# iden3/circom

Measured on NVIDIA H100. Metric: witnesses/s, higher is better.
Workload: dtype u256 (8x u32 limbs, Montgomery)

## Files before the change

### circom_b200/csrc/flatten.cpp

```cpp
#include <algorithm>
#include <bitset>
#include <cstdio>
#include <cstdlib>
#include <cstring>
#include <functional>
#include <stdexcept>
#include <unordered_map>

#include "../../include/circom_b200.h"
#include "tape.h"

namespace cw {

uint64_t fnv1a(const char *s, size_t n) {
    uint64_t h = 0xCBF29CE484222325ULL;
    for (size_t i = 0; i < n; ++i) {
        h ^= (uint64_t)(int64_t)(signed char)s[i];
        h *= 0x100000001B3ULL;
    }
    return h;
}

namespace {

enum { K_NONE = 0, K_OWN = 1, K_SUB = 2, K_CONST = 3, K_TMP = 4, K_ONE = 5 };
enum Form { FC = 0, FM = 1, FD = 2 };

struct IrOp {
    uint32_t op;
    uint64_t d, a, b, c;
};
struct Term {
    uint64_t ref;
    uint32_t cid;
};
struct Tmpl {
    std::string name;
    uint32_t n_out, n_in, n_inter, n_tmp, n_own;
    std::vector<uint32_t> subs;
    std::vector<IrOp> ops;
    std::vector<uint32_t> lc_len;
    std::vector<Term> terms;
    std::vector<uint8_t> tmp_zero_only;
    uint64_t total_signals = 0, total_components = 0;
};

inline int rk(uint64_t r) { return (int)(r >> 56); }
inline uint32_t rsub(uint64_t r) { return (uint32_t)((r >> 32) & 0xFFFFFF); }
inline uint32_t ridx(uint64_t r) { return (uint32_t)r; }

struct Reader {
    const uint8_t *p, *end;
    template <class T>
    T get() {
        if (p + sizeof(T) > end) throw std::runtime_error("cb2c: truncated");
        T v;
        memcpy(&v, p, sizeof(T));
        p += sizeof(T);
        return v;
    }
    const uint8_t *bytes(size_t n) {
        if (n > (size_t)(end - p)) throw std::runtime_error("cb2c: truncated");
        const uint8_t *r = p;
        p += n;
        return r;
    }
    size_t left() const { return (size_t)(end - p); }
    void expect(uint64_t count, uint64_t bytes_each) const {
        if (count * bytes_each > left()) throw std::runtime_error("cb2c: truncated (count exceeds the file)");
    }
    std::string str() {
        uint32_t n = get<uint32_t>();
        const uint8_t *b = bytes((size_t)(((uint64_t)n + 3) & ~3ull));
        return std::string((const char *)b, n);
    }
};

struct Val {
    uint32_t slot[3] = {NO_SLOT, NO_SLOT, NO_SLOT};
    int32_t cid = -1;
    uint16_t bits = 256;
    uint8_t org_op = 0;
    int32_t org_a = -1, org_b = -1;
    int32_t fld_src = -1, bf_src = -1;
    uint16_t fld_k = 0, fld_m = 0, bf_lo = 0, bf_len = 0;
};

enum { DOP_BITS = 29, DOP_ASSERT_BOOL = 30, DOP_MULSMALL = 31, DOP_BITSIP = 32, DOP_ASSERT_FITS = 33 };
enum { DOP_ADDI = 48, DOP_SHRK = 49, DOP_SHLK = 50, DOP_ADDI_H = 52, DOP_MULI_Q = 53, DOP_MULI_H = 54, DOP_SHRK_H = 55,
       DOP_SHLK_H = 56 };
inline bool c_is_immediate(uint32_t opcode) {
    return opcode == CW_OP_ASSERT || opcode == CW_OP_ASSERT_EQ || opcode == DOP_BITS || opcode == DOP_ASSERT_BOOL ||
           opcode == DOP_BITSIP || opcode == DOP_ASSERT_FITS;
}
inline bool is_assert_op(uint32_t opcode) {
    return opcode == CW_OP_ASSERT || opcode == CW_OP_ASSERT_EQ || opcode == DOP_ASSERT_BOOL || opcode == DOP_ASSERT_FITS;
}

inline size_t n_live_ops(const std::vector<uint8_t> &live, uint32_t n_pre, size_t n_prov) {
    size_t n = 0;
    for (size_t i = 0; i < n_prov; ++i) n += live[n_pre + i];
    return n;
}
inline int subtree_need(uint32_t i, const std::vector<uint32_t> &kid_a, const std::vector<uint32_t> &kid_b) {
    const uint32_t a = kid_a[i], b = kid_b[i];
    if (a == NO_SLOT && b == NO_SLOT) return 1;
    if (a == NO_SLOT) return subtree_need(b, kid_a, kid_b);
    if (b == NO_SLOT) return subtree_need(a, kid_a, kid_b);
    const int na = subtree_need(a, kid_a, kid_b), nb = subtree_need(b, kid_a, kid_b);
    return std::max(std::max(na, nb), std::min(na, nb) + 1);
}

static uint32_t coalesce_function_copies(uint32_t *code, uint32_t n_instr, uint32_t n_regs, const std::vector<uint32_t> &fn_params) {
    constexpr uint32_t MAXR = 192;
    if (n_regs > MAXR || n_instr < 2) return n_instr;
    using Set = std::bitset<MAXR>;
    enum { JMP = 40, JZ = 41, RET = 42, LOADX = 43, STOREX = 44, CALLF = 45, COPY = 24 };
    auto is_reg = [&](uint32_t o) { return !(o & 0xC0000000u) && o < n_regs; };
    Set pinned;
    std::vector<uint8_t> target(n_instr + 1, 0);
    for (uint32_t i = 0; i < n_instr; ++i) {
        const uint32_t *w = &code[5 * (size_t)i];
        uint32_t lo = 0, hi = 0;
        if (w[0] == LOADX) { lo = w[2] & 0x3FFFFFFFu; hi = w[4] & 0x3FFFFFFFu; }
        else if (w[0] == STOREX) { lo = w[2] & 0x3FFFFFFFu; hi = w[1] & 0x3FFFFFFFu; }
        else if (w[0] == RET && (w[3] & 0x3FFFFFFFu) > 1) { lo = w[2]; hi = lo + (w[3] & 0x3FFFFFFFu); }
        else if (w[0] == CALLF) {
            for (uint32_t r = w[3]; r < w[3] + fn_params[w[2] & 0x3FFFFFFFu] && r < n_regs; ++r) pinned.set(r);
            if ((w[4] & 0x3FFFFFFFu) > 1) { lo = w[1]; hi = lo + (w[4] & 0x3FFFFFFFu); }
        }
        for (uint32_t r = lo; r < hi && r < n_regs; ++r) pinned.set(r);
        if (w[0] == JMP) target[std::min(w[2] & 0x3FFFFFFFu, n_instr)] = 1;
        if (w[0] == JZ) target[std::min(w[3] & 0x3FFFFFFFu, n_instr)] = 1;
    }
    std::vector<Set> use(n_instr), live_in(n_instr), live_out(n_instr);
    std::vector<int> def(n_instr, -1);
    auto add_use = [&](uint32_t i, uint32_t o) { if (is_reg(o) && !pinned.test(o)) use[i].set(o); };
    for (uint32_t i = 0; i < n_instr; ++i) {
        const uint32_t *w = &code[5 * (size_t)i];
        switch (w[0]) {
            case JMP: break;
            case JZ: add_use(i, w[2]); break;
            case RET: if ((w[3] & 0x3FFFFFFFu) <= 1) add_use(i, w[2]); break;
            case LOADX: add_use(i, w[3]); if (!pinned.test(w[1])) def[i] = (int)w[1]; break;
            case STOREX: add_use(i, w[3]); add_use(i, w[4]); break;
            case CALLF: if (!pinned.test(w[1])) def[i] = (int)w[1]; break;
            default: add_use(i, w[2]); add_use(i, w[3]); add_use(i, w[4]); if (!pinned.test(w[1])) def[i] = (int)w[1];
        }
    }
    for (bool changed = true; changed;) {
        changed = false;
        for (uint32_t i = n_instr; i-- > 0;) {
            const uint32_t *w = &code[5 * (size_t)i];
            Set out;
            if (w[0] == JMP) out = live_in[w[2] & 0x3FFFFFFFu];
            else if (w[0] != RET) {
                if (i + 1 < n_instr) out = live_in[i + 1];
                if (w[0] == JZ) out |= live_in[w[3] & 0x3FFFFFFFu];
            }
            Set in = out;
            if (def[i] >= 0) in.reset((size_t)def[i]);
            in |= use[i];
            if (in != live_in[i] || out != live_out[i]) { live_in[i] = in; live_out[i] = out; changed = true; }
        }
    }
    std::vector<uint8_t> dead(n_instr, 0);
    for (uint32_t i = 1; i < n_instr; ++i) {
        uint32_t *c = &code[5 * (size_t)i], *p = &code[5 * (size_t)(i - 1)];
        if (c[0] != COPY || target[i] || dead[i - 1]) continue;
        const uint32_t t = c[2], d = c[1];
        if (!is_reg(t) || pinned.test(t) || t == d || def[i - 1] != (int)t || live_out[i].test(t)) continue;
        if (p[0] == JMP || p[0] == JZ || p[0] == RET || p[0] == STOREX) continue;
// ... 1349 lines not shown
                }
                ext[i] = e;
                gsig[i] = sg * 1099511628211ull;
                if (!fusedf[i]) {
                    glevel[n_pre + i] = e + 1;
                    max_level = std::max(max_level, e + 1);
                    ++n_roots;
                }
            }
        }
        std::vector<uint32_t> order;
        order.reserve(n_roots);
        for (size_t i = 0; i < n_prov; ++i)
            if (live[n_pre + i] && !fusedf[i] && pops[i * 4] != 47) order.push_back((uint32_t)i);
        std::stable_sort(order.begin(), order.end(), [&](uint32_t x, uint32_t y) {
            uint32_t lx = glevel[n_pre + x], ly = glevel[n_pre + y];
            if (lx != ly) return lx < ly;
            if (pops[x * 4] != pops[y * 4]) return pops[x * 4] < pops[y * 4];
            return gsig[x] < gsig[y];
        });
        std::vector<uint32_t> remap(n_pre + n_prov, NO_SLOT);
        uint32_t next_tmp = (uint32_t)W;
        for (uint32_t i = 0; i < n_pre; ++i) {
            if (claimed[i] < 0) throw std::runtime_error("lowering: main input outside the witness");
            remap[i] = (uint32_t)claimed[i];
        }
        for (size_t r = 0; r < order.size(); ++r) {
            uint32_t p = n_pre + order[r];
            if (claimed[p] >= 0) remap[p] = (uint32_t)claimed[p];
            else if (!is_assert_op(pops[(size_t)order[r] * 4])) remap[p] = next_tmp++;
            if (pops[(size_t)order[r] * 4] == 45) {
                const uint32_t *ct = &pcalls[pops[(size_t)order[r] * 4 + 1]];
                const uint32_t *ex = ct + 2 + ct[1];
                for (uint32_t k = 0; k < ex[0]; ++k) {
                    const uint32_t s = ex[1 + k];
                    if (!live[s]) continue;
                    remap[s] = claimed[s] >= 0 ? (uint32_t)claimed[s] : next_tmp++;
                }
            }
        }
        if (next_tmp >= DST_ACC) throw std::runtime_error("circuit too large for the packed tape word (2^24 slots)");
        T.ops.clear();
        T.ops.reserve(n_live_ops(live, n_pre, n_prov) * 4);
        T.items.clear();
        T.items.reserve(n_roots + 1);
        T.level_start.assign(max_level + 1, 0);
        T.n_mul_ops = 0;
        uint32_t prev_level = 0;
        const bool narrow_on = !(flags & (CW_FLAG_NO_NARROW | CW_FLAG_NO_PEEPHOLE));
        auto opd_bits = [&](uint32_t o) -> uint32_t {
            if (o == NO_SLOT) return 0;
            if (o & OPERAND_CONST) return (uint32_t)u256_bitlen(consts[o & 0x7FFFFFFFu]);
            return o < slot_bits.size() ? slot_bits[o] : 256u;
        };
        auto const_amount = [&](uint32_t o, uint32_t &k) {
            if (o == NO_SLOT || !(o & OPERAND_CONST)) return false;
            const U256 &c = consts[o & 0x7FFFFFFFu];
            if (c.v[1] | c.v[2] | c.v[3] || c.v[0] >= qb()) return false;
            k = (uint32_t)c.v[0];
            return true;
        };
        auto narrow_opcode = [&](uint32_t i) -> uint32_t {
            const uint32_t *o = &pops[(size_t)i * 4];
            if (!narrow_on) return o[0];
            const uint32_t rb = slot_bits[n_pre + i], ba = opd_bits(o[1]), bb = opd_bits(o[2]), lim = qb() - 1;
            uint32_t k;
            switch (o[0]) {
                case CW_OP_ADD:
                    if (rb >= 256 || std::max(ba, bb) + 1 > lim) return o[0];
                    return std::max(ba, bb) + 1 <= 128 ? DOP_ADDI_H : DOP_ADDI;
                case DOP_MULSMALL:
                    if (ba <= 64 && bb <= 64) return DOP_MULI_Q;
                    if (ba <= 128 && bb <= 128) return DOP_MULI_H;
                    return o[0];
                case CW_OP_SHR:
                    if (!const_amount(o[2], k)) return o[0];
                    return ba <= 128 ? DOP_SHRK_H : DOP_SHRK;
                case CW_OP_SHL:
                    if (!const_amount(o[2], k) || ba + k > lim) return o[0];
                    return ba <= 128 ? DOP_SHLK_H : DOP_SHLK;
                default: return o[0];
            }
        };
        for (uint64_t &x : T.width_census) x = 0;
        auto census = [&](uint32_t i, uint32_t opcode) {
            const uint32_t *o = &pops[(size_t)i * 4];
            uint32_t w = is_assert_op(o[0]) ? 0u : slot_bits[n_pre + i];
            for (int k = 1; k <= 3; ++k) {
                if (k == 3 && c_is_immediate(o[0])) break;
                if (o[k] != NO_SLOT && !(o[k] & OPERAND_CONST)) w = std::max(w, opd_bits(o[k]));
            }
            T.width_census[4 * (opcode & 63u) + (w <= 64 ? 0 : w <= 128 ? 1 : w <= 192 ? 2 : 3)]++;
        };
        auto word = [&](uint32_t i, uint32_t dstfield, int acc_a, int acc_b, uint32_t d[4]) {
            const uint32_t *o = &pops[(size_t)i * 4];
            const uint32_t opcode = o[0] == 45 ? o[0] : narrow_opcode(i);
            d[0] = opcode | (dstfield << 8);
            if (o[0] == 45) {
                uint32_t n = pcalls[o[1] + 1];
                d[1] = (uint32_t)T.call_tab.size();
                d[2] = d[3] = OPERAND_CONST;
                T.call_tab.push_back(pcalls[o[1]]);
                T.call_tab.push_back(n);
                for (uint32_t k = 0; k < n; ++k) {
                    uint32_t a = pcalls[o[1] + 2 + k];
                    T.call_tab.push_back((a & OPERAND_CONST) ? a : remap[a]);
                }
                const uint32_t *ex = &pcalls[o[1] + 2 + n];
                T.call_tab.push_back(ex[0]);
                for (uint32_t k = 0; k < ex[0]; ++k) T.call_tab.push_back(live[ex[1 + k]] ? remap[ex[1 + k]] : NO_SLOT);
                return;
            }
            for (int k = 1; k <= 3; ++k) {
                if (k == 3 && c_is_immediate(o[0])) d[k] = o[k];
                else if (o[k] == NO_SLOT) d[k] = OPERAND_CONST;
                else if (o[k] & OPERAND_CONST) d[k] = o[k];
                else if (k == 1 && acc_a >= 0) d[k] = OPERAND_ACC | (uint32_t)acc_a;
                else if (k == 2 && acc_b >= 0) d[k] = OPERAND_ACC | (uint32_t)acc_b;
                else d[k] = remap[o[k]];
            }
        };
        std::function<void(uint32_t, int)> emit_sub = [&](uint32_t i, int target) {
            const uint32_t ka = kid_a[i], kb = kid_b[i];
            int acc_a = -1, acc_b = -1;
            if (ka != NO_SLOT && kb != NO_SLOT) {
                const bool a_first = subtree_need(ka, kid_a, kid_b) >= subtree_need(kb, kid_a, kid_b);
                if (a_first) { emit_sub(ka, target); emit_sub(kb, target ^ 1); }
                else { emit_sub(kb, target); emit_sub(ka, target ^ 1); }
                acc_a = a_first ? target : (target ^ 1);
                acc_b = a_first ? (target ^ 1) : target;
            } else if (ka != NO_SLOT) { emit_sub(ka, target); acc_a = target; }
            else if (kb != NO_SLOT) { emit_sub(kb, target); acc_b = target; }
            uint32_t d[4];
            word(i, DST_ACC + (uint32_t)target, acc_a, acc_b, d);
            census(i, d[0] & 0xFFu);
            T.ops.insert(T.ops.end(), d, d + 4);
            if (pops[(size_t)i * 4] == CW_OP_MUL) ++T.n_mul_ops;
        };
        for (size_t r = 0; r < order.size(); ++r) {
            const uint32_t i = order[r];
            const uint32_t *o = &pops[(size_t)i * 4];
            const uint32_t lvl = glevel[n_pre + i];
            const uint32_t dst = is_assert_op(o[0]) ? 0u : remap[n_pre + i];
            const uint32_t ka = kid_a[i], kb = kid_b[i];
            const bool single = ka == NO_SLOT && kb == NO_SLOT;
            uint32_t d[4];
            if (single) {
                word(i, dst, -1, -1, d);
                if (o[0] == DOP_BITS && !(flags & CW_FLAG_NO_PEEPHOLE) && lvl == prev_level && !T.ops.empty() &&
                    T.items.back() == T.ops.size() / 4 - 1) {
                    uint32_t *p = &T.ops[T.ops.size() - 4];
                    if ((p[0] & 0xFFu) == DOP_BITS && p[1] == d[1] && ((p[3] >> 16) & 0xFFu) == 1u && ((d[3] >> 16) & 0xFFu) == 1u) {
                        uint32_t cnt = (p[3] >> 24) + 1u, pk = p[3] & 0xFFFFu, pdst = p[0] >> 8;
                        if (cnt < 32u && (d[3] & 0xFFFFu) == pk + cnt && dst == pdst + cnt) {
                            p[3] += 1u << 24;
                            continue;
                        }
                    }
                }
                if (o[0] != 45) census(i, d[0] & 0xFFu);
                T.items.push_back((uint32_t)(T.ops.size() / 4));
                T.ops.insert(T.ops.end(), d, d + 4);
            } else {
                T.items.push_back((uint32_t)(T.ops.size() / 4));
                int acc_a = -1, acc_b = -1;
                if (ka != NO_SLOT && kb != NO_SLOT) {
                    const bool a_first = subtree_need(ka, kid_a, kid_b) >= subtree_need(kb, kid_a, kid_b);
                    if (a_first) { emit_sub(ka, 0); emit_sub(kb, 1); }
                    else { emit_sub(kb, 0); emit_sub(ka, 1); }
                    acc_a = a_first ? 0 : 1;
                    acc_b = a_first ? 1 : 0;
                } else if (ka != NO_SLOT) { emit_sub(ka, 0); acc_a = 0; }
                else { emit_sub(kb, 0); acc_b = 0; }
                word(i, dst, acc_a, acc_b, d);
                census(i, d[0] & 0xFFu);
                T.ops.insert(T.ops.end(), d, d + 4);
            }
            prev_level = lvl;
            if (o[0] == CW_OP_MUL) ++T.n_mul_ops;
            T.level_start[lvl]++;
        }
        T.items.push_back((uint32_t)(T.ops.size() / 4));
        {
            std::vector<uint32_t> ls(max_level + 1, 0);
            uint32_t acc = 0;
            uint64_t widest = 0;
            for (uint32_t l = 1; l <= max_level; ++l) {
                ls[l - 1] = acc;
                widest = std::max<uint64_t>(widest, T.level_start[l]);
                acc += T.level_start[l];
            }
            ls[max_level] = acc;
            T.level_start.swap(ls);
            T.max_level_width = widest;
        }
        std::vector<uint32_t> newid;
        T.n_bitwords = 0;
        if (flags & CW_FLAG_BITPLANE) {
            std::vector<uint32_t> code(next_tmp, NO_SLOT);
            uint32_t n_words = 0;
            const size_t n_ops = T.ops.size() / 4;
            for (size_t i = 0; i < n_ops; ++i) {
                const uint32_t *o = &T.ops[i * 4];
                if ((o[0] & 0xFFu) != DOP_BITS || !(o[3] >> 24)) continue;
                const uint32_t run = (o[3] >> 24) + 1u, d0 = o[0] >> 8;
                for (uint32_t j = 0; j < run; ++j) code[d0 + j] = OPERAND_BIT | (n_words * 32u + j);
                ++n_words;
            }
            bool ok = n_words > 0 && n_words < (1u << 24);
            for (size_t i = 0; ok && i < n_ops; ++i) {
                const uint32_t *o = &T.ops[i * 4];
                if ((o[0] & 0xFFu) == DOP_BITS && (o[3] >> 24) && !(o[1] & OPERAND_CONST) && code[o[1]] != NO_SLOT) ok = false;
            }
            for (uint32_t i = 0; ok && i < M.n_in + 1; ++i)
                if (code[remap[i]] != NO_SLOT) ok = false;
            if (next_tmp >= OPERAND_BIT) ok = false;
            if (ok) {
                newid.resize(next_tmp);
                uint32_t nw = 0;
                for (uint32_t s = 0; s < next_tmp; ++s) newid[s] = code[s] == NO_SLOT ? nw++ : code[s];
                uint32_t word = 0;
                for (size_t i = 0; i < n_ops; ++i) {
                    uint32_t *o = &T.ops[i * 4];
                    const uint32_t opc = o[0] & 0xFFu;
                    if (opc == DOP_BITS && (o[3] >> 24)) o[0] = opc | (word++ << 8);
                    else if (!is_assert_op(opc) && (o[0] >> 8) < DST_ACC) o[0] = opc | (newid[o[0] >> 8] << 8);
                    if (opc == 45) continue;
                    for (int k = 1; k <= 3; ++k) {
                        if (k == 3 && c_is_immediate(opc)) break;
                        if (!(o[k] & (OPERAND_CONST | OPERAND_ACC))) o[k] = newid[o[k]];
                    }
                }
                for (size_t i = 0; i < T.call_tab.size();) {
                    const uint32_t n = T.call_tab[i + 1], nx = T.call_tab[i + 2 + n];
                    for (uint32_t k = 0; k < n + 1 + nx; ++k) {
                        if (k == n) continue;
                        uint32_t &e = T.call_tab[i + 2 + k];
                        if (!(e & OPERAND_CONST)) e = newid[e];
                    }
                    i += 3 + n + nx;
                }
                T.n_bitwords = n_words;
                next_tmp = nw;
            }
        }
        const uint32_t n_resident = newid.empty() ? (uint32_t)W : [&]() {
            uint32_t n = 0;
            for (uint64_t i = 0; i < W; ++i) n += !(newid[i] & OPERAND_BIT);
            return n;
        }();
        if (flags & CW_FLAG_REUSE) {
            const size_t n_ops = T.ops.size() / 4;
            const size_t n_lv = T.level_start.size() - 1;
            std::vector<uint32_t> last(next_tmp, 0), phys(next_tmp, NO_SLOT);
            auto is_tmp = [&](uint32_t o) { return !(o & (OPERAND_CONST | OPERAND_BIT | OPERAND_ACC)) && o >= n_resident; };
            for (size_t l = 0; l < n_lv; ++l)
                for (uint32_t i = T.items[T.level_start[l]]; i < T.items[T.level_start[l + 1]]; ++i) {
                    const uint32_t *o = &T.ops[(size_t)i * 4];
                    const uint32_t opc = o[0] & 0xFFu;
                    if (opc == 45) {
                        const uint32_t n = T.call_tab[o[1] + 1];
                        for (uint32_t k = 0; k < n; ++k)
                            if (is_tmp(T.call_tab[o[1] + 2 + k])) last[T.call_tab[o[1] + 2 + k]] = (uint32_t)l;
                        continue;
                    }
// ... 79 lines not shown
        }
        T.witness_slot.resize(W);
        for (uint64_t i = 0; i < W; ++i) T.witness_slot[i] = newid.empty() ? (uint32_t)i : newid[i];
        T.input_slot.resize(M.n_in);
        for (uint32_t i = 0; i < M.n_in; ++i) T.input_slot[i] = newid.empty() ? remap[1 + i] : newid[remap[1 + i]];
        if (remap[0] != 0) throw std::runtime_error("lowering: constant-one signal is not witness entry 0");
        T.consts = consts;
        if (T.consts.empty()) T.consts.push_back(u256_from_u64(0));
        T.dat_consts = ir_consts;
        for (int k = 0; k < 4; ++k) T.slot_census[k] = 0;
        for (size_t i = 0; i < n_pre + n_prov; ++i) {
            if (remap[i] == NO_SLOT) continue;
            const uint16_t b = slot_bits[i];
            T.slot_census[b <= 1 ? 0 : b <= 32 ? 1 : b <= 64 ? 2 : 3]++;
        }
        T.n_pre = n_pre;
        T.n_slots = next_tmp;
        T.n_ir_ops = n_ir_ops;
        T.n_conv_ops = n_conv;
        T.n_asserts = n_asserts;
        T.flags = flags;
        for (const Tmpl &t : tm) T.tmpl_names.push_back(t.name);

        uint64_t hs = 256;
        while (hs < T.inputs.size()) hs <<= 1;
        T.hashmap.assign(hs, HashEntry{0, 0, 0});
        for (const InputInfo &in : T.inputs) {
            uint64_t p = in.hash % hs;
            while (T.hashmap[p].signalid != 0) p = (p + 1) % hs;
            T.hashmap[p] = HashEntry{in.hash, in.signal_id, in.size};
        }

    }
};

}

void lower_circuit(const uint8_t *data, size_t len, uint32_t flags, Tape &out) {
    Lowerer L(out, flags);
    L.parse(data, len);
    L.lower();
}

}

namespace cw {
namespace {
struct BlobW {
    std::vector<uint8_t> &o;
    void raw(const void *p, size_t n) { o.insert(o.end(), (const uint8_t *)p, (const uint8_t *)p + n); }
    template <class T> void pod(const T &v) { raw(&v, sizeof(T)); }
    template <class T> void vec(const std::vector<T> &v) {
        pod<uint64_t>(v.size());
        if (!v.empty()) raw(v.data(), v.size() * sizeof(T));
    }
    void str(const std::string &s) {
        pod<uint64_t>(s.size());
        raw(s.data(), s.size());
    }
};
struct BlobR {
    const uint8_t *p, *end;
    void raw(void *d, size_t n) {
        if (n > (size_t)(end - p)) throw std::runtime_error("lowered-circuit blob: truncated");
        memcpy(d, p, n);
        p += n;
    }
    template <class T> void pod(T &v) { raw(&v, sizeof(T)); }
    template <class T> void vec(std::vector<T> &v) {
        uint64_t n;
        pod(n);
        if (n > (uint64_t)(end - p) / sizeof(T)) throw std::runtime_error("lowered-circuit blob: bad length");
        v.resize(n);
        if (n) raw(v.data(), n * sizeof(T));
    }
    void str(std::string &s) {
        uint64_t n;
        pod(n);
        if (n > (uint64_t)(end - p)) throw std::runtime_error("lowered-circuit blob: bad length");
        s.assign((const char *)p, n);
        p += n;
    }
};
constexpr uint32_t BLOB_VERSION = 7;
}

void serialize_tape(const Tape &t, std::vector<uint8_t> &out) {
    BlobW w{out};
    w.raw("CB2T", 4);
    w.pod<uint32_t>(BLOB_VERSION);
    w.pod<int32_t>(t.F.prime_id);
    w.pod(t.flags);
    const uint64_t nums[] = {t.n_signals, t.n_witness, t.n_inputs, t.n_outputs, t.n_components, t.n_ir_ops, t.n_mul_ops,
                             t.n_conv_ops, t.max_level_width, t.n_asserts, t.slot_census[0], t.slot_census[1],
                             t.slot_census[2], t.slot_census[3], t.n_slot_operands, t.n_values, t.n_resident, t.n_pre,
                             t.n_slots, t.n_bitwords, t.n_stored};
    w.pod<uint64_t>(sizeof(nums) / 8);
    w.raw(nums, sizeof(nums));
    w.vec(t.ops); w.vec(t.items); w.vec(t.level_start); w.vec(t.consts); w.vec(t.dat_consts); w.vec(t.witness_slot); w.vec(t.input_slot);
    w.vec(t.pk_bit_wire); w.vec(t.pk_u64_wire); w.vec(t.pk_full_wire); w.vec(t.wit_class); w.vec(t.wit_bits);
    w.vec(t.fn_code); w.vec(t.fn_info); w.vec(t.call_tab); w.vec(t.witness2signal);
    w.raw(t.width_census, sizeof(t.width_census));
    w.pod<uint64_t>(t.inputs.size());
    for (const InputInfo &in : t.inputs) {
        w.str(in.name);
        w.pod(in.hash); w.pod(in.signal_id); w.pod(in.size);
    }
    w.vec(t.hashmap);
    const R1csData &r = t.r1cs;
    w.pod<int32_t>(r.prime_id);
    w.pod(r.n_wires); w.pod(r.n_constraints);
    w.vec(r.row_ptr); w.vec(r.col); w.vec(r.coef); w.vec(r.dict);
    w.pod(r.n_pub_out); w.pod(r.n_pub_in); w.pod(r.n_prv_in);
}

void deserialize_tape(const uint8_t *data, size_t len, Tape &t) {
    BlobR r{data, data + len};
    char magic[4];
    r.raw(magic, 4);
    uint32_t ver;
    r.pod(ver);
    if (memcmp(magic, "CB2T", 4) || ver != BLOB_VERSION) throw std::runtime_error("lowered-circuit blob: bad magic / version");
    int32_t prime;
    r.pod(prime);
    if (prime < 0 || prime >= CW_N_PRIMES) throw std::runtime_error("lowered-circuit blob: unknown prime");
    t.F = make_field(prime);
    r.pod(t.flags);
    uint64_t n_nums;
    r.pod(n_nums);
    uint64_t nums[21];
    if (n_nums != 21) throw std::runtime_error("lowered-circuit blob: layout mismatch");
    r.raw(nums, sizeof(nums));
    t.n_signals = nums[0]; t.n_witness = nums[1]; t.n_inputs = nums[2]; t.n_outputs = nums[3]; t.n_components = nums[4];
    t.n_ir_ops = nums[5]; t.n_mul_ops = nums[6]; t.n_conv_ops = nums[7]; t.max_level_width = nums[8]; t.n_asserts = nums[9];
    for (int k = 0; k < 4; ++k) t.slot_census[k] = nums[10 + k];
    t.n_slot_operands = nums[14]; t.n_values = nums[15]; t.n_resident = (uint32_t)nums[16]; t.n_pre = (uint32_t)nums[17];
    t.n_slots = (uint32_t)nums[18]; t.n_bitwords = (uint32_t)nums[19]; t.n_stored = nums[20];
    r.vec(t.ops); r.vec(t.items); r.vec(t.level_start); r.vec(t.consts); r.vec(t.dat_consts); r.vec(t.witness_slot); r.vec(t.input_slot);
    r.vec(t.pk_bit_wire); r.vec(t.pk_u64_wire); r.vec(t.pk_full_wire); r.vec(t.wit_class); r.vec(t.wit_bits);
    r.vec(t.fn_code); r.vec(t.fn_info); r.vec(t.call_tab); r.vec(t.witness2signal);
    r.raw(t.width_census, sizeof(t.width_census));
    uint64_t n_in;
    r.pod(n_in);
    if (n_in > len) throw std::runtime_error("lowered-circuit blob: bad length");
    t.inputs.resize(n_in);
    for (InputInfo &in : t.inputs) {
        r.str(in.name);
        r.pod(in.hash); r.pod(in.signal_id); r.pod(in.size);
    }
    r.vec(t.hashmap);
    R1csData &R = t.r1cs;
    int32_t rp;
    r.pod(rp);
    R.prime_id = rp;
    r.pod(R.n_wires); r.pod(R.n_constraints);
    r.vec(R.row_ptr); r.vec(R.col); r.vec(R.coef); r.vec(R.dict);
    r.pod(R.n_pub_out); r.pod(R.n_pub_in); r.pod(R.n_prv_in);
    if (t.ops.size() % 4 || t.level_start.empty() || t.items.empty() || t.level_start.back() != t.items.size() - 1 ||
        t.items.back() != t.ops.size() / 4 ||
        t.witness_slot.size() != t.n_witness || t.input_slot.size() != t.n_inputs || t.wit_class.size() != t.n_witness || t.wit_bits.size() != t.n_witness ||
        t.witness2signal.size() != t.n_witness || R.row_ptr.size() != 3 * R.n_constraints + 1 || R.col.size() != R.coef.size() ||
        (R.row_ptr.size() && R.row_ptr.back() != R.col.size()) || t.hashmap.empty())
        throw std::runtime_error("lowered-circuit blob: inconsistent");
}

}
```

### circom_b200/csrc/fr_device.cuh

```cuda
#pragma once
#include <stddef.h>
#include <stdint.h>

#if defined(__CUDACC__)
#define CW_HD __host__ __device__ __forceinline__
#else
#define CW_HD inline
#endif

namespace cw {

typedef uint32_t u32;
typedef uint64_t u64;

struct FrParams {
    u32 q[8];
    u32 half[8];
    u32 r1[8];
    u32 r2[8];
    u32 qm2[8];
    u32 np32;
    u32 qbits;
    u32 top_mask;
    u32 pad;
// ... 494 lines not shown
            if (a[i]) {
                u32 x = a[i], c = 0;
                while (!(x & 0x80000000u)) { x <<= 1; ++c; }
                n += c;
                done = true;
            } else n += 32;
        }
    }
    return n;
}
CW_HD bool u256_divmod(u32 *quo, u32 *rem, const u32 *a, const u32 *b) {
    if (u256_is_zero(b)) {
        u256_set_u32(quo, 0);
        u256_set_u32(rem, 0);
        return false;
    }
    u32 lzb = u256_clz(b);
    {
        u32 single[8], one[8];
        u256_set_u32(one, 1);
        u256_shl(single, one, 255 - lzb);
        if (u256_eq(single, b)) {
            u32 bit = 255 - lzb;
            u256_shr(quo, a, bit);
            u32 t[8];
            u256_shl(t, quo, bit);
            u256_sub(rem, a, t);
            return true;
        }
    }
    u32 lza = u256_clz(a);
    u32 n[8], q[8], r[8];
    if (lza == 256) {
        u256_set_u32(quo, 0);
        u256_set_u32(rem, 0);
        return true;
    }
    u256_shl(n, a, lza);
    u256_set_u32(q, 0);
    u256_set_u32(r, 0);
    int steps = 256 - (int)lza;
#if defined(__CUDA_ARCH__)
#pragma unroll 1
#endif
    for (int i = 0; i < steps; ++i) {
        u32 carry = n[7] >> 31;
#pragma unroll
        for (int j = 7; j > 0; --j) n[j] = (n[j] << 1) | (n[j - 1] >> 31);
        n[0] <<= 1;
        const u32 rtop = r[7] >> 31;
#pragma unroll
        for (int j = 7; j > 0; --j) r[j] = (r[j] << 1) | (r[j - 1] >> 31);
        r[0] = (r[0] << 1) | carry;
        u32 t[8];
        u32 br = u256_sub(t, r, b);
#pragma unroll
        for (int j = 7; j > 0; --j) q[j] = (q[j] << 1) | (q[j - 1] >> 31);
        q[0] <<= 1;
        if (rtop || !br) {
            u256_set(r, t);
            q[0] |= 1;
        }
    }
    u256_set(quo, q);
    u256_set(rem, r);
    return true;
}

enum {
    OP_MUL = 1, OP_ADD = 3, OP_SUB = 4, OP_POW = 5, OP_IDIV = 6, OP_MOD = 7, OP_SHL = 8, OP_SHR = 9,
    OP_LEQ = 10, OP_GEQ = 11, OP_LT = 12, OP_GT = 13, OP_EQ = 14, OP_NEQ = 15, OP_LOR = 16, OP_LAND = 17,
    OP_LNOT = 18, OP_BOR = 19, OP_BAND = 20, OP_BXOR = 21, OP_BNOT = 22, OP_NEG = 23, OP_COPY = 24,
    OP_SELECT = 25, OP_ASSERT = 26, OP_ASSERT_EQ = 27, OP_INV = 28,
    OP_BITS = 29,
    OP_ASSERT_BOOL = 30,
    OP_MULSMALL = 31,
    OP_BITSIP = 32,
    OP_ASSERT_FITS = 33
};
enum {
    OP_ADDI = 48,
    OP_SHRK = 49,
    OP_SHLK = 50,
    OP_NARROW_HALF = 52,
    OP_ADDI_H = 52,
    OP_MULI_Q = 53,
    OP_MULI_H = 54,
    OP_SHRK_H = 55,
    OP_SHLK_H = 56
};

CW_HD void u256_mul_lo(u32 *r, const u32 *a, const u32 *b) {
    u32 t[8];
#pragma unroll
    for (int i = 0; i < 8; ++i) t[i] = 0;
#pragma unroll
    for (int i = 0; i < 8; ++i) {
        u64 c = 0;
#pragma unroll
        for (int j = 0; j + i < 8; ++j) {
            c += (u64)a[j] * b[i] + t[i + j];
            t[i + j] = (u32)c;
            c >>= 32;
        }
    }
    u256_set(r, t);
}
template <int N>
CW_HD void u256_mul_narrow(u32 *r, const u32 *a, const u32 *b) {
    u32 t[8];
#pragma unroll
    for (int i = 0; i < 8; ++i) t[i] = 0;
#pragma unroll
    for (int i = 0; i < N; ++i) {
        u64 c = 0;
#pragma unroll
        for (int j = 0; j < N; ++j) {
            c += (u64)a[j] * b[i] + t[i + j];
            t[i + j] = (u32)c;
            c >>= 32;
        }
        t[i + N] = (u32)c;
    }
    u256_set(r, t);
}
CW_HD void u128_add(u32 *r, const u32 *a, const u32 *b) {
#if defined(__CUDA_ARCH__)
    u32 r0, r1, r2, r3;
    asm("add.cc.u32 %0, %4, %8;\n\t"
        "addc.cc.u32 %1, %5, %9;\n\t"
        "addc.cc.u32 %2, %6, %10;\n\t"
        "addc.u32 %3, %7, %11;"
        : "=&r"(r0), "=&r"(r1), "=&r"(r2), "=&r"(r3)
        : "r"(a[0]), "r"(a[1]), "r"(a[2]), "r"(a[3]), "r"(b[0]), "r"(b[1]), "r"(b[2]), "r"(b[3]));
    r[0] = r0; r[1] = r1; r[2] = r2; r[3] = r3;
#else
    u64 c = 0;
    for (int i = 0; i < 4; ++i) {
        c += (u64)a[i] + b[i];
        r[i] = (u32)c;
        c >>= 32;
    }
#endif
    r[4] = r[5] = r[6] = r[7] = 0;
}
CW_HD void u256_low_half(u32 *r, const u32 *a) {
    r[0] = a[0]; r[1] = a[1]; r[2] = a[2]; r[3] = a[3];
    r[4] = r[5] = r[6] = r[7] = 0;
}
CW_HD void u256_bits(u32 *r, const u32 *a, u32 imm) {
    u32 k = imm & 0xFFFFu, m = (imm >> 16) & 0xFFu;
    u32 t[8];
    u256_shr(t, a, k);
#pragma unroll
    for (int i = 0; i < 8; ++i) {
        int lo = i * 32;
        u32 mask = (int)m >= lo + 32 ? 0xFFFFFFFFu : ((int)m <= lo ? 0u : ((1u << (m - lo)) - 1u));
        r[i] = t[i] & mask;
    }
}

CW_HD void u256_bits_in_place(u32 *r, const u32 *a, u32 imm) {
    u32 lo = imm & 0xFFu, len = imm >> 8, hi = lo + len;
#pragma unroll
    for (int i = 0; i < 8; ++i) {
        u32 b0 = 32u * i, b1 = b0 + 32u;
        u32 m = 0;
        if (hi > b0 && lo < b1) {
            u32 from = lo > b0 ? lo - b0 : 0u, to = hi < b1 ? hi - b0 : 32u;
            u32 w = to - from;
            m = (w >= 32u ? 0xFFFFFFFFu : ((1u << w) - 1u)) << from;
        }
        r[i] = a[i] & m;
    }
}
CW_HD u32 u256_bitlen(const u32 *a) {
    u32 n = 0;
#pragma unroll
    for (int i = 0; i < 8; ++i) {
        if (a[i]) {
            u32 x = a[i], c = 0;
            while (x) { x >>= 1; ++c; }
            n = 32u * i + c;
        }
    }
    return n;
}

template <bool SLOW>
CW_HD void fr_exec_t(u32 opcode, u32 *r, const u32 *a, const u32 *b, u32 imm, const FrParams &P, int &err) {
    switch (opcode) {
        case OP_BITSIP: u256_bits_in_place(r, a, imm); break;
        case OP_BITS: u256_bits(r, a, imm); break;
        case OP_MULSMALL: u256_mul_lo(r, a, b); break;
        case OP_MUL: fr_mont_mul(r, a, b, P); break;
        case OP_ADD: fr_add(r, a, b, P); break;
        case OP_SUB: fr_sub(r, a, b, P); break;
        case OP_NEG: fr_neg(r, a, P); break;
        case OP_INV: if (SLOW) fr_inv_mont(r, a, P); break;
        case OP_POW: if (SLOW) fr_pow_mont(r, a, b, P); break;
        case OP_IDIV: { u32 rem[8]; if (!u256_divmod(r, rem, a, b)) err = 1; break; }
        case OP_MOD: { u32 quo[8]; if (!u256_divmod(quo, r, a, b)) err = 1; break; }
        case OP_SHL: fr_shl(r, a, b, P); break;
        case OP_SHR: fr_shr(r, a, b, P); break;
        case OP_LT: u256_set_u32(r, fr_lt(a, b, P)); break;
        case OP_GT: u256_set_u32(r, fr_lt(b, a, P)); break;
        case OP_LEQ: u256_set_u32(r, !fr_lt(b, a, P)); break;
        case OP_GEQ: u256_set_u32(r, !fr_lt(a, b, P)); break;
        case OP_EQ: u256_set_u32(r, u256_eq(a, b)); break;
        case OP_NEQ: u256_set_u32(r, !u256_eq(a, b)); break;
        case OP_LOR: u256_set_u32(r, !u256_is_zero(a) || !u256_is_zero(b)); break;
        case OP_LAND: u256_set_u32(r, !u256_is_zero(a) && !u256_is_zero(b)); break;
        case OP_LNOT: u256_set_u32(r, u256_is_zero(a)); break;
        case OP_BOR:
#pragma unroll
            for (int i = 0; i < 8; ++i) r[i] = a[i] | b[i];
            fr_mask_wrap(r, P);
            break;
        case OP_BAND:
#pragma unroll
            for (int i = 0; i < 8; ++i) r[i] = a[i] & b[i];
            fr_mask_wrap(r, P);
            break;
        case OP_BXOR:
#pragma unroll
            for (int i = 0; i < 8; ++i) r[i] = a[i] ^ b[i];
            fr_mask_wrap(r, P);
            break;
        case OP_BNOT:
#pragma unroll
            for (int i = 0; i < 8; ++i) r[i] = ~a[i];
            fr_mask_wrap(r, P);
            break;
        case OP_COPY: u256_set(r, a); break;
        case OP_ADDI: u256_add(r, a, b); break;
        case OP_SHRK: u256_shr(r, a, b[0]); break;
        case OP_SHLK: u256_shl(r, a, b[0]); break;
        case OP_ADDI_H: u128_add(r, a, b); break;
        case OP_MULI_Q: u256_mul_narrow<2>(r, a, b); break;
        case OP_MULI_H: u256_mul_narrow<4>(r, a, b); break;
        case OP_SHRK_H: { u32 t[8]; u256_low_half(t, a); u256_shr(r, t, b[0]); break; }
        case OP_SHLK_H: { u32 t[8]; u256_low_half(t, a); u256_shl(r, t, b[0]); break; }
        default: u256_set_u32(r, 0); break;
    }
}
CW_HD void fr_exec(u32 opcode, u32 *r, const u32 *a, const u32 *b, u32 imm, const FrParams &P, int &err) {
    fr_exec_t<true>(opcode, r, a, b, imm, P, err);
}

CW_HD void fr_apply_canonical(u32 op, u32 *r, const u32 *a, const u32 *b, const u32 *c, const FrParams &P, int &err) {
    if (op == OP_MUL) {
        if (u256_bitlen(a) + u256_bitlen(b) < P.qbits) {
            u256_mul_lo(r, a, b);
        } else {
            u32 am[8];
            fr_to_mont(am, a, P);
            fr_mont_mul(r, am, b, P);
        }
    } else if (op == 2 ) {
        u32 bm[8], im[8];
        fr_to_mont(bm, b, P);
        fr_inv_mont(im, bm, P);
        fr_mont_mul(r, im, a, P);
    } else if (op == OP_POW) {
        u32 am[8], rm[8];
        fr_to_mont(am, a, P);
        fr_pow_mont(rm, am, b, P);
        fr_from_mont(r, rm, P);
    } else if (op == OP_SELECT) {
        bool t = !u256_is_zero(c);
        for (int k = 0; k < 8; ++k) r[k] = t ? a[k] : b[k];
    } else {
        fr_exec(op, r, a, b, 0, P, err);
    }
}

enum { FOP_JMP = 40, FOP_JZ = 41, FOP_RET = 42, FOP_LOADX = 43, FOP_STOREX = 44, OP_CALL = 45 };
enum { VM_MAX_REGS = 192, VM_MAX_STEPS = 1 << 22, VM_MAX_DEPTH = 8 };
struct FnInfo {
    u32 code_off, n_instr, n_regs, n_params;
};
CW_HD FnInfo vm_fn(const u32 *fn_info, u32 f) {
    FnInfo fi;
    fi.code_off = fn_info[4 * (size_t)f];
    fi.n_instr = fn_info[4 * (size_t)f + 1];
    fi.n_regs = fn_info[4 * (size_t)f + 2];
    fi.n_params = fn_info[4 * (size_t)f + 3];
    return fi;
}
struct VmFrame {
    u32 fn, pc, base, dst, want;
};

CW_HD void vm_operand(u32 *v, u32 o, const u32 *regs, const u32 *consts32) {
    if (o & 0x80000000u) {
        const u32 *p = consts32 + 8 * (size_t)(o & 0x3FFFFFFFu);
        for (int k = 0; k < 8; ++k) v[k] = p[k];
    } else if (o & 0x40000000u) {
        u256_set_u32(v, o & 0x3FFFFFFFu);
    } else {
        const u32 *p = regs + 8 * (size_t)o;
        for (int k = 0; k < 8; ++k) v[k] = p[k];
    }
}
CW_HD int vm_index(const u32 *v, u32 base, u32 limit) {
    u32 hi = v[1] | v[2] | v[3] | v[4] | v[5] | v[6] | v[7];
    if (hi || (u64)v[0] + base >= limit) return -1;
    return (int)(v[0] + base);
}
#if defined(__CUDACC__)
__host__ __device__
#endif
inline void vm_run(const u32 *code, const u32 *fn_info, u32 fn, u32 *regs, const u32 *consts32, u32 *result, const FrParams &P,
                   int &err, u32 &ret_base, u32 &ret_cnt) {
    FnInfo fi = vm_fn(fn_info, fn);
    const u32 *ins = code + 5 * (size_t)fi.code_off;
    u32 *fr = regs;
    u32 base = 0, depth = 0;
    VmFrame stack[VM_MAX_DEPTH];
    u32 pc = 0;
// ... 267 lines not shown
```

### circom_b200/csrc/u256.h

```cpp
#pragma once
#include <cstdint>
#include <cstring>
#include <string>

namespace cw {

struct U256 {
    uint64_t v[4];
    bool operator==(const U256 &o) const { return !memcmp(v, o.v, 32); }
    bool operator!=(const U256 &o) const { return !(*this == o); }
    bool operator<(const U256 &o) const {
        for (int i = 3; i >= 0; --i) {
            if (v[i] != o.v[i]) return v[i] < o.v[i];
        }
        return false;
    }
    bool is_zero() const { return (v[0] | v[1] | v[2] | v[3]) == 0; }
};

inline U256 u256_from_u64(uint64_t x) { return U256{{x, 0, 0, 0}}; }

inline uint64_t u256_add(U256 &r, const U256 &a, const U256 &b) {
    unsigned __int128 c = 0;
    for (int i = 0; i < 4; ++i) {
        c += (unsigned __int128)a.v[i] + b.v[i];
        r.v[i] = (uint64_t)c;
        c >>= 64;
    }
    return (uint64_t)c;
}
inline uint64_t u256_sub(U256 &r, const U256 &a, const U256 &b) {
    unsigned __int128 br = 0;
    for (int i = 0; i < 4; ++i) {
        unsigned __int128 t = (unsigned __int128)a.v[i] - b.v[i] - br;
        r.v[i] = (uint64_t)t;
        br = (t >> 64) & 1;
    }
    return (uint64_t)br;
}

constexpr int CW_N_PRIMES = 8;
int prime_id_of(const struct U256 &q);

struct FieldParams {
    int prime_id;
    U256 q;
    U256 half;
    U256 r1;
    U256 r2;
    uint64_t np64;
    uint32_t np32;
    uint32_t qbits;

    U256 addm(const U256 &a, const U256 &b) const {
        U256 r;
        uint64_t c = u256_add(r, a, b);
        if (c || !(r < q)) u256_sub(r, r, q);
        return r;
    }
    U256 subm(const U256 &a, const U256 &b) const {
        U256 r;
        if (u256_sub(r, a, b)) u256_add(r, r, q);
        return r;
    }
    U256 mont_mul(const U256 &a, const U256 &b) const {
        uint64_t t[6] = {0, 0, 0, 0, 0, 0};
        for (int i = 0; i < 4; ++i) {
            unsigned __int128 c = 0;
            for (int j = 0; j < 4; ++j) {
                c += (unsigned __int128)a.v[j] * b.v[i] + t[j];
                t[j] = (uint64_t)c;
                c >>= 64;
            }
            c += t[4];
            t[4] = (uint64_t)c;
            t[5] = (uint64_t)(c >> 64);
            uint64_t m = t[0] * np64;
            c = (unsigned __int128)m * q.v[0] + t[0];
            c >>= 64;
            for (int j = 1; j < 4; ++j) {
                c += (unsigned __int128)m * q.v[j] + t[j];
                t[j - 1] = (uint64_t)c;
                c >>= 64;
            }
            c += t[4];
            t[3] = (uint64_t)c;
            t[4] = t[5] + (uint64_t)(c >> 64);
        }
        U256 r{{t[0], t[1], t[2], t[3]}};
        if (t[4] || !(r < q)) u256_sub(r, r, q);
        return r;
    }
    U256 to_mont(const U256 &a) const { return mont_mul(a, r2); }
    U256 from_mont(const U256 &a) const { return mont_mul(a, u256_from_u64(1)); }
    U256 mulm(const U256 &a, const U256 &b) const { return mont_mul(to_mont(a), b); }
};

inline FieldParams make_field(int prime_id) {
    FieldParams f;
    f.prime_id = prime_id;
    static const uint64_t Q[CW_N_PRIMES][4] = {
        {0x43e1f593f0000001ULL, 0x2833e84879b97091ULL, 0xb85045b68181585dULL, 0x30644e72e131a029ULL},
        {0xffffffff00000001ULL, 0x53bda402fffe5bfeULL, 0x3339d80809a1d805ULL, 0x73eda753299d7d48ULL},
        {0x3c208c16d87cfd47ULL, 0x97816a916871ca8dULL, 0xb85045b68181585dULL, 0x30644e72e131a029ULL},
        {0x992d30ed00000001ULL, 0x224698fc094cf91bULL, 0x0000000000000000ULL, 0x4000000000000000ULL},
        {0x8c46eb2100000001ULL, 0x224698fc0994a8ddULL, 0x0000000000000000ULL, 0x4000000000000000ULL},
        {0xffffffffffffffffULL, 0x00000000ffffffffULL, 0x0000000000000000ULL, 0xffffffff00000001ULL},
        {0x0a11800000000001ULL, 0x59aa76fed0000001ULL, 0x60b44d1e5c37b001ULL, 0x12ab655e9a2ca556ULL},
        {0xffffffff00000001ULL, 0x0000000000000000ULL, 0x0000000000000000ULL, 0x0000000000000000ULL},
    };
    memcpy(f.q.v, Q[prime_id >= 0 && prime_id < CW_N_PRIMES ? prime_id : 0], 32);
    for (int i = 0; i < 4; ++i) f.half.v[i] = (f.q.v[i] >> 1) | (i < 3 ? (f.q.v[i + 1] << 63) : 0);
    uint64_t inv = 1;
    for (int i = 0; i < 6; ++i) inv *= 2 - f.q.v[0] * inv;
    f.np64 = (uint64_t)(0 - inv);
    f.np32 = (uint32_t)f.np64;
    int bits = 0;
    for (int i = 255; i >= 0; --i) {
        if ((f.q.v[i / 64] >> (i % 64)) & 1) { bits = i + 1; break; }
    }
    f.qbits = bits;
    U256 x = u256_from_u64(1);
    for (int i = 0; i < 512; ++i) {
        x = f.addm(x, x);
        if (i == 255) f.r1 = x;
    }
    f.r2 = x;
    return f;
}

inline int prime_id_of(const U256 &q) {
    for (int i = 0; i < CW_N_PRIMES; ++i)
        if (make_field(i).q == q) return i;
    return -1;
}

}
```

Before: 201,300.

## Replace Montgomery multiply by small constants with Barrett-reduced narrow multiply

At tape flatten time, multiplications whose constant operand has a canonical value below 2^64 (or exactly 2^64) are rewritten to a new MULK opcode. The constant operand carries the raw small value plus a precomputed Barrett factor. On the device a 256x64-bit product is reduced with a single Barrett step and up to two conditional subtractions, in place of a full 8x8-limb Montgomery multiply. The rewrite applies only to primes wider than 224 bits, changes the tape blob version, and adds an optional census printout.

Result: faster. 227,400, median of 6 (+13.0%).

```diff
diff --git a/circom_b200/csrc/flatten.cpp b/circom_b200/csrc/flatten.cpp
--- a/circom_b200/csrc/flatten.cpp
+++ b/circom_b200/csrc/flatten.cpp
@@ -87,7 +87,7 @@
 };
 
 enum { DOP_BITS = 29, DOP_ASSERT_BOOL = 30, DOP_MULSMALL = 31, DOP_BITSIP = 32, DOP_ASSERT_FITS = 33 };
-enum { DOP_ADDI = 48, DOP_SHRK = 49, DOP_SHLK = 50, DOP_ADDI_H = 52, DOP_MULI_Q = 53, DOP_MULI_H = 54, DOP_SHRK_H = 55,
+enum { DOP_ADDI = 48, DOP_SHRK = 49, DOP_SHLK = 50, DOP_MULK = 51, DOP_ADDI_H = 52, DOP_MULI_Q = 53, DOP_MULI_H = 54, DOP_SHRK_H = 55,
        DOP_SHLK_H = 56 };
 inline bool c_is_immediate(uint32_t opcode) {
     return opcode == CW_OP_ASSERT || opcode == CW_OP_ASSERT_EQ || opcode == DOP_BITS || opcode == DOP_ASSERT_BOOL ||
@@ -1603,6 +1603,25 @@
                 default: return o[0];
             }
         };
+        struct MulK { uint32_t cls, operand; };
+        std::unordered_map<uint32_t, MulK> mulk_of;
+        const bool mulk_prime = F.qbits > 224;
+        const uint64_t mu = mulk_prime ? F.barrett_mu() : 0;
+        auto mulk = [&](uint32_t i) -> MulK {
+            const uint32_t *o = &pops[(size_t)i * 4];
+            if (o[0] != CW_OP_MUL || o[2] == NO_SLOT || !(o[2] & OPERAND_CONST)) return MulK{0, NO_SLOT};
+            const uint32_t K = o[2] & 0x7FFFFFFFu;
+            auto it = mulk_of.find(K);
+            if (it != mulk_of.end()) return it->second;
+            const U256 k = F.from_mont(consts[K]);
+            MulK r{3, NO_SLOT};
+            if (!(k.v[1] | k.v[2] | k.v[3])) r.cls = k.v[0] >> 32 ? 2 : 1;
+            else if (k.v[1] == 1 && !k.v[0] && !(k.v[2] | k.v[3])) r.cls = 2;
+            if (r.cls < 3 && mulk_prime) r.operand = OPERAND_CONST | raw_const(U256{{k.v[0], k.v[1], mu, 0}});
+            mulk_of.emplace(K, r);
+            return r;
+        };
+        uint64_t mul_census[4] = {0, 0, 0, 0};
         for (uint64_t &x : T.width_census) x = 0;
         auto census = [&](uint32_t i, uint32_t opcode) {
             const uint32_t *o = &pops[(size_t)i * 4];
@@ -1615,7 +1634,8 @@
         };
         auto word = [&](uint32_t i, uint32_t dstfield, int acc_a, int acc_b, uint32_t d[4]) {
             const uint32_t *o = &pops[(size_t)i * 4];
-            const uint32_t opcode = o[0] == 45 ? o[0] : narrow_opcode(i);
+            const MulK mk = mulk(i);
+            const uint32_t opcode = o[0] == 45 ? o[0] : (narrow_on && mk.operand != NO_SLOT) ? DOP_MULK : narrow_opcode(i);
             d[0] = opcode | (dstfield << 8);
             if (o[0] == 45) {
                 uint32_t n = pcalls[o[1] + 1];
@@ -1640,6 +1660,7 @@
                 else if (k == 2 && acc_b >= 0) d[k] = OPERAND_ACC | (uint32_t)acc_b;
                 else d[k] = remap[o[k]];
             }
+            if (opcode == DOP_MULK) d[2] = mk.operand;
         };
         std::function<void(uint32_t, int)> emit_sub = [&](uint32_t i, int target) {
             const uint32_t ka = kid_a[i], kb = kid_b[i];
@@ -1656,7 +1677,7 @@
             word(i, DST_ACC + (uint32_t)target, acc_a, acc_b, d);
             census(i, d[0] & 0xFFu);
             T.ops.insert(T.ops.end(), d, d + 4);
-            if (pops[(size_t)i * 4] == CW_OP_MUL) ++T.n_mul_ops;
+            if (pops[(size_t)i * 4] == CW_OP_MUL) { ++T.n_mul_ops; ++mul_census[mulk(i).cls]; }
         };
         for (size_t r = 0; r < order.size(); ++r) {
             const uint32_t i = order[r];
@@ -1698,10 +1719,15 @@
                 T.ops.insert(T.ops.end(), d, d + 4);
             }
             prev_level = lvl;
-            if (o[0] == CW_OP_MUL) ++T.n_mul_ops;
+            if (o[0] == CW_OP_MUL) { ++T.n_mul_ops; ++mul_census[mulk(i).cls]; }
             T.level_start[lvl]++;
         }
         T.items.push_back((uint32_t)(T.ops.size() / 4));
+        if (const char *cenv = getenv("CW_FUSION_CENSUS"); cenv && atoi(cenv))
+            fprintf(stderr, "product census: Montgomery products by the canonical value k of their constant operand: "
+                    "no constant %llu, k < 2^32 %llu, 2^32 <= k <= 2^64 %llu, wider %llu\n",
+                    (unsigned long long)mul_census[0], (unsigned long long)mul_census[1], (unsigned long long)mul_census[2],
+                    (unsigned long long)mul_census[3]);
         {
             std::vector<uint32_t> ls(max_level + 1, 0);
             uint32_t acc = 0;
@@ -1947,7 +1973,7 @@
         p += n;
     }
 };
-constexpr uint32_t BLOB_VERSION = 7;
+constexpr uint32_t BLOB_VERSION = 8;
 }
 
 void serialize_tape(const Tape &t, std::vector<uint8_t> &out) {
diff --git a/circom_b200/csrc/fr_device.cuh b/circom_b200/csrc/fr_device.cuh
--- a/circom_b200/csrc/fr_device.cuh
+++ b/circom_b200/csrc/fr_device.cuh
@@ -600,6 +600,7 @@
     OP_ADDI = 48,
     OP_SHRK = 49,
     OP_SHLK = 50,
+    OP_MULK = 51,
     OP_NARROW_HALF = 52,
     OP_ADDI_H = 52,
     OP_MULI_Q = 53,
@@ -607,6 +608,81 @@
     OP_SHRK_H = 55,
     OP_SHLK_H = 56
 };
+
+CW_HD u64 u64_mul_hi(u64 x, u64 y) {
+#if defined(__CUDA_ARCH__)
+    return __umul64hi(x, y);
+#else
+    return (u64)(((unsigned __int128)x * y) >> 64);
+#endif
+}
+CW_HD void fr_mul_small(u32 *r, const u32 *a, const u32 *kb, const FrParams &P) {
+    u32 t[10];
+    if (kb[2]) {
+        t[0] = t[1] = 0;
+#pragma unroll
+        for (int j = 0; j < 8; ++j) t[j + 2] = a[j];
+    } else {
+        u64 c = 0;
+#pragma unroll
+        for (int j = 0; j < 8; ++j) {
+            c += (u64)a[j] * kb[0];
+            t[j] = (u32)c;
+            c >>= 32;
+        }
+        t[8] = (u32)c;
+        c = 0;
+#pragma unroll
+        for (int j = 0; j < 8; ++j) {
+            c += (u64)a[j] * kb[1] + t[j + 1];
+            t[j + 1] = (u32)c;
+            c >>= 32;
+        }
+        t[9] = (u32)c;
+    }
+    const u32 sh = (P.qbits - 1u) & 31u;
+    const u64 t1 = ((((u64)t[8] << 32) | t[7]) >> sh) | ((u64)((((u64)t[9] << 32) | t[8]) >> sh) << 32);
+    const u32 t1_top = t[9] >> sh;
+    const u64 m = (u64)kb[4] | ((u64)kb[5] << 32);
+    u64 x = u64_mul_hi(t1, m), y;
+    u32 cx = t1_top;
+    y = x + t1;
+    cx += y < x;
+    x = y + (t1_top ? m : 0ull);
+    cx += x < y;
+    const u64 qh = (x >> 1) | ((u64)cx << 63);
+    u32 p[9];
+    {
+        const u32 q0 = (u32)qh, q1 = (u32)(qh >> 32);
+        u64 c = 0;
+#pragma unroll
+        for (int j = 0; j < 8; ++j) {
+            c += (u64)P.q[j] * q0;
+            p[j] = (u32)c;
+            c >>= 32;
+        }
+        p[8] = (u32)c;
+        c = 0;
+#pragma unroll
+        for (int j = 0; j < 7; ++j) {
+            c += (u64)P.q[j] * q1 + p[j + 1];
+            p[j + 1] = (u32)c;
+            c >>= 32;
+        }
+        p[8] += (u32)c + P.q[7] * q1;
+    }
+    u32 br = u256_sub(r, t, p);
+    u32 r8 = t[8] - p[8] - br;
+#pragma unroll
+    for (int k = 0; k < 2; ++k) {
+        u32 d[8];
+        br = u256_sub(d, r, P.q);
+        const bool keep = r8 < br;
+#pragma unroll
+        for (int i = 0; i < 8; ++i) r[i] = keep ? r[i] : d[i];
+        r8 = keep ? r8 : r8 - br;
+    }
+}
 
 CW_HD void u256_mul_lo(u32 *r, const u32 *a, const u32 *b) {
     u32 t[8];
@@ -754,6 +830,7 @@
         case OP_ADDI: u256_add(r, a, b); break;
         case OP_SHRK: u256_shr(r, a, b[0]); break;
         case OP_SHLK: u256_shl(r, a, b[0]); break;
+        case OP_MULK: fr_mul_small(r, a, b, P); break;
         case OP_ADDI_H: u128_add(r, a, b); break;
         case OP_MULI_Q: u256_mul_narrow<2>(r, a, b); break;
         case OP_MULI_H: u256_mul_narrow<4>(r, a, b); break;
diff --git a/circom_b200/csrc/u256.h b/circom_b200/csrc/u256.h
--- a/circom_b200/csrc/u256.h
+++ b/circom_b200/csrc/u256.h
@@ -94,6 +94,19 @@
     U256 to_mont(const U256 &a) const { return mont_mul(a, r2); }
     U256 from_mont(const U256 &a) const { return mont_mul(a, u256_from_u64(1)); }
     U256 mulm(const U256 &a, const U256 &b) const { return mont_mul(to_mont(a), b); }
+    uint64_t barrett_mu() const {
+        U256 rem = u256_from_u64(1);
+        uint64_t quo = 0;
+        for (uint32_t i = 0; i < qbits + 64; ++i) {
+            const uint64_t carry = u256_add(rem, rem, rem);
+            quo <<= 1;
+            if (carry || !(rem < q)) {
+                u256_sub(rem, rem, q);
+                quo |= 1;
+            }
+        }
+        return quo;
+    }
 };
 
 inline FieldParams make_field(int prime_id) {
```
